# jameshensman/pyvb

Measured on AMD Instinct MI355X. Metric: VB update iterations/sec (T=10k, D=64, N=1024 LDS); ELBO rel-err vs NumPy, higher is better.
Workload: dtype f64; 1 GPU; LDS T=10000 D=64 K=64, 1024 replicates per GPU (BASELINE configs[2]); replicates_total=1024, parallelism=replicates sharded over 1 GPU(s), collective=none (1 GPU), degraded=False

## Files before the change

### pyvb_amd/csrc/k_cols.hip

```cpp
#include "params.h"

#define MFMA(a, b, c) __builtin_amdgcn_mfma_f64_16x16x4f64((a), (b), (c), 0, 0, 0)
#define MS 72
#define GS 68

__device__ __forceinline__ void load_row16(const double* row, int col0, int D, bool vec, double fill, double* out) {
    if (vec) {
#pragma unroll
        for (int g = 0; g < 4; ++g) {
            if (col0 + 4 * g < D) {
                const d4 v = *reinterpret_cast<const d4*>(row + col0 + 4 * g);
                out[4 * g] = v[0]; out[4 * g + 1] = v[1]; out[4 * g + 2] = v[2]; out[4 * g + 3] = v[3];
            } else {
                out[4 * g] = out[4 * g + 1] = out[4 * g + 2] = out[4 * g + 3] = fill;
            }
        }
    } else {
#pragma unroll
        for (int u = 0; u < 16; ++u) {
            const int c = col0 + u;
            const double v = row[c < D ? c : D - 1];
            out[u] = c < D ? v : fill;
        }
    }
}

__global__ void __launch_bounds__(64) k_cols(ParamArgs a) {
    const int WHICH = a.which0 + blockIdx.y;
    __shared__ double Mb[64 * MS];
    __shared__ double Gb[16 * GS];
    __shared__ double Sb[16 * GS];
    const int n = blockIdx.x, lane = threadIdx.x, D = a.D, K = a.K, c = lane & 15, q = lane >> 4;
    if (!a.active[n]) return;
    const int rows = WHICH == 0 ? D : K;
    double* M = (WHICH == 0 ? a.A_mean : a.C_mean) + (size_t)n * rows * D;
    double* V = (WHICH == 0 ? a.A_var : a.C_var) + (size_t)n * D * rows;
    double* qld = (WHICH == 0 ? a.qld_A : a.qld_C) + (size_t)n * D;
    double* lnd = (WHICH == 0 ? a.lnd_A : a.lnd_C) + (size_t)n * D;
    const double* pm = WHICH == 0 ? a.pri.A_pm : a.pri.C_pm;
    const double* pp = WHICH == 0 ? a.pri.A_pp : a.pri.C_pp;
    const double* obs = WHICH == 0 ? a.pri.A_obs : a.pri.C_obs;
    const double* mo = a.mom + (size_t)n * mom_total(D, K);
    const double* G = mo + (WHICH == 0 ? MOM_GA(D, K) : MOM_GC(D, K));
    const double* H = mo + (WHICH == 0 ? MOM_HA(D, K) : MOM_HC(D, K));
    const bool live = lane < rows;
    const int lr = live ? lane : 0;
    const int lc = lane < D ? lane : D - 1;
    const bool vec = (D & 3) == 0;
    const int nb = (D + 15) >> 4;
    const double* Mrow = M + (size_t)lr * D;
    const double* Hrow = H + (size_t)lr * D;

    for (int b = 0; b < 4; ++b) {
        double m[16] = {};
        if (b < nb) load_row16(Mrow, 16 * b, D, vec, 0.0, m);
#pragma unroll
        for (int u = 0; u < 16; ++u) Mb[(16 * b + u) * MS + lane] = (b < nb && live) ? m[u] : 0.0;
    }
    const double lam = live ? (WHICH == 0 ? a.Q_a[(size_t)n * D + lane] / a.Q_b[(size_t)n * D + lane]
                                          : a.R_a[(size_t)n * K + lane] / a.R_b[(size_t)n * K + lane]) : 0.0;

    auto stage_G = [&](int b) {
        double g[16];
#pragma unroll
        for (int u = 0; u < 16; ++u) {
            const int i = 16 * b + u;
            g[u] = G[(size_t)(i < D ? i : D - 1) * D + lc];
        }
#pragma unroll
        for (int u = 0; u < 16; ++u) Gb[u * GS + lane] = (16 * b + u < D && lane < D) ? g[u] : 0.0;
    };
    auto product = [&]() {
        d4 acc[4];
#pragma unroll
        for (int rt = 0; rt < 4; ++rt) acc[rt] = d4{0.0, 0.0, 0.0, 0.0};
#pragma unroll 4
        for (int s = 0; s < 16; ++s) {
            const double bop = Gb[c * GS + 4 * s + q];
#pragma unroll
            for (int rt = 0; rt < 4; ++rt) acc[rt] = MFMA(Mb[(4 * s + q) * MS + 16 * rt + c], bop, acc[rt]);
        }
#pragma unroll
        for (int rt = 0; rt < 4; ++rt)
#pragma unroll
            for (int r = 0; r < 4; ++r) Sb[c * GS + 16 * rt + 4 * r + q] = acc[rt][r];
    };

    if (a.c0 < a.c1) {
        for (int b = a.c0 >> 4; b <= (a.c1 - 1) >> 4; ++b) {
            __syncthreads();
            stage_G(b);
            double p0[16], m0[16], hk[16], ob[16];
#pragma unroll
            for (int u = 0; u < 16; ++u) {
                const int i = 16 * b + u;
                p0[u] = pp[(size_t)(i < D ? i : D - 1) * rows + lr];
            }
            load_row16(pm + (size_t)lr * D, 16 * b, D, vec, 0.0, m0);
            load_row16(Hrow, 16 * b, D, vec, 0.0, hk);
            load_row16(obs + (size_t)lr * D, 16 * b, D, vec, 0.0, ob);
            __syncthreads();
            product();
            __syncthreads();
            double gd[16], var[16], base[16];
#pragma unroll
            for (int u = 0; u < 16; ++u) {
                gd[u] = Gb[u * GS + 16 * b + u];
                const double prec = p0[u] + lam * gd[u];
                var[u] = 1.0 / prec;
                base[u] = p0[u] * m0[u] + lam * hk[u];
                p0[u] = prec;
            }
            double dl[16];
            int mynk = 0;
#pragma unroll
            for (int u = 0; u < 16; ++u) {
                const int i = 16 * b + u;
                dl[u] = 0.0;
                if (i >= a.c0 && i < a.c1) {
                    const double xo = Mb[i * MS + lane];
                    double acc = Sb[u * GS + lane] - xo * gd[u];
#pragma unroll
                    for (int v = 0; v < u; ++v) acc += dl[v] * Gb[u * GS + 16 * b + v];
                    double val = (base[u] - lam * acc) * var[u], vr = var[u];
                    const bool known = live && (ob[u] == ob[u]);
                    if (known) { val = ob[u]; vr = 0.0; }
                    const int nknown = __popcll(__ballot(known));
                    mynk = (lane == u) ? nknown : mynk;
                    if (live) {
                        dl[u] = val - xo;
                        Mb[i * MS + lane] = val;
                        V[(size_t)i * rows + lane] = vr;
                    }
                    Sb[u * GS + lane] = live ? p0[u] : 1.0;
                } else {
                    Sb[u * GS + lane] = 1.0;
                    mynk = (lane == u) ? rows : mynk;
                }
            }
            __syncthreads();
            {
                double mant = 1.0; int ex = 0;
#pragma unroll
                for (int r = 0; r < 16; ++r) {
                    int e;
                    mant *= frexp(Sb[c * GS + 16 * q + r], &e);
                    ex += e;
                }
#pragma unroll
                for (int o = 16; o <= 32; o <<= 1) {
                    mant *= __shfl_xor(mant, o, 64);
                    ex += __shfl_xor(ex, o, 64);
                }
                const int i = 16 * b + c;
                if (q == 0 && i >= a.c0 && i < a.c1 && mynk < rows) {
                    const double lp = log(mant) + (double)ex * 0.6931471805599453;
                    qld[i] = 0.5 / (0.5 * lp);
                    lnd[i] = -lp;
                }
            }
        }
        __syncthreads();
        if (live) {
            for (int b = a.c0 >> 4; b <= (a.c1 - 1) >> 4; ++b) {
#pragma unroll
                for (int g = 0; g < 4; ++g) {
                    const int cc = 16 * b + 4 * g;
                    if (vec) {
                        if (cc < D) {
                            d4 v;
#pragma unroll
                            for (int r = 0; r < 4; ++r) v[r] = Mb[(cc + r) * MS + lane];
                            *reinterpret_cast<d4*>(M + (size_t)lane * D + cc) = v;
                        }
                    } else {
#pragma unroll
                        for (int r = 0; r < 4; ++r)
                            if (cc + r < D) M[(size_t)lane * D + cc + r] = Mb[(cc + r) * MS + lane];
                    }
                }
            }
        }
    }

    if (a.fuse & 1) {
        double e0 = 0.0, e1 = 0.0, hm0 = 0.0, hm1 = 0.0;
        for (int b = 0; b < nb; ++b) {
            __syncthreads();
            stage_G(b);
            double hk[16], vv[16];
            load_row16(Hrow, 16 * b, D, vec, 0.0, hk);
#pragma unroll
            for (int u = 0; u < 16; ++u) {
                const int i = 16 * b + u;
                vv[u] = V[(size_t)(i < D ? i : D - 1) * rows + lr];
            }
            __syncthreads();
            product();
            __syncthreads();
#pragma unroll
            for (int u = 0; u < 16; u += 2) {
                const int i = 16 * b + u;
                const double x0 = Mb[i * MS + lane], x1 = Mb[(i + 1) * MS + lane];
                e0 += x0 * Sb[u * GS + lane] + (i < D ? vv[u] * Gb[u * GS + i] : 0.0);
                e1 += x1 * Sb[(u + 1) * GS + lane] + (i + 1 < D ? vv[u + 1] * Gb[(u + 1) * GS + i + 1] : 0.0);
                hm0 += x0 * hk[u];
                hm1 += x1 * hk[u + 1];
            }
        }
        const double own = WHICH == 0 ? mo[MOM_DP(D, K) + lr] : a.Syy[(size_t)n * K + lr];
        double r = 0.5 * own + 0.5 * (e0 + e1) - (hm0 + hm1);
        if (live) (WHICH == 0 ? a.resQ : a.resR)[(size_t)n * rows + lane] = r;
        if (a.fuse & 2) {
            const double* b0 = WHICH == 0 ? a.pri.Q_b0 : a.pri.R_b0;
            double* qb = (WHICH == 0 ? a.Q_b : a.R_b) + (size_t)n * rows;
            r = live ? r : 0.0;
            if (a.noise == PYVB_NOISE_GAMMA) {
                r = wave_sum(r);
                if (live) qb[lane] = b0[0] + r;
            } else if (live) {
                qb[lane] = b0[lane] + r;
            }
        }
    }
}

int launch_cols(pyvb_lds* h, int which, int c0, int c1, int fuse) {
    if (h->big) return launch_cols_big(h, which, c0, c1, fuse);
    ParamArgs a = make_args(h);
    a.c0 = c0; a.c1 = c1; a.which0 = which == 1 ? 1 : 0; a.fuse = fuse;
    TimedLaunch tl(h, PYVB_K_PARAMS);
    hipLaunchKernelGGL(k_cols, dim3(h->N, which == 2 ? 2 : 1), dim3(64), 0, h->stream, a);
    HIPCHK(hipGetLastError());
    return PYVB_OK;
}

int launch_resid(pyvb_lds* h, int which) { return launch_cols(h, which, 0, 0, 1); }
```

Before: 87.57 VB iterations/s per 1024 replicates (whole job).

## Hold mean matrix in MFMA-operand registers, staging only a 16-column tile in LDS

The full 64x64 mean matrix now lives in per-lane registers laid out as MFMA A operands, instead of a 64-row LDS buffer. Only the current 16-column block is copied into a small LDS tile for the sequential coordinate update, then copied back into registers and written to global memory per block. This cuts LDS use (more blocks per CU) and replaces LDS operand reads in the matrix product with register reads. The cost is 64 extra VGPRs per lane, register select logic in to_tile/from_tile, and a fully unrolled product loop, which may raise register pressure or cause spills.

Result: no change. 88.40 VB iterations/s per 1024 replicates (whole job), median of 6 (+1.0%).

```diff
diff --git a/pyvb_amd/csrc/k_cols.hip b/pyvb_amd/csrc/k_cols.hip
--- a/pyvb_amd/csrc/k_cols.hip
+++ b/pyvb_amd/csrc/k_cols.hip
@@ -27,7 +27,7 @@
 
 __global__ void __launch_bounds__(64) k_cols(ParamArgs a) {
     const int WHICH = a.which0 + blockIdx.y;
-    __shared__ double Mb[64 * MS];
+    __shared__ double Tb[16 * MS];
     __shared__ double Gb[16 * GS];
     __shared__ double Sb[16 * GS];
     const int n = blockIdx.x, lane = threadIdx.x, D = a.D, K = a.K, c = lane & 15, q = lane >> 4;
@@ -48,15 +48,36 @@
     const int lc = lane < D ? lane : D - 1;
     const bool vec = (D & 3) == 0;
     const int nb = (D + 15) >> 4;
-    const double* Mrow = M + (size_t)lr * D;
     const double* Hrow = H + (size_t)lr * D;
 
-    for (int b = 0; b < 4; ++b) {
-        double m[16] = {};
-        if (b < nb) load_row16(Mrow, 16 * b, D, vec, 0.0, m);
-#pragma unroll
-        for (int u = 0; u < 16; ++u) Mb[(16 * b + u) * MS + lane] = (b < nb && live) ? m[u] : 0.0;
-    }
+    double Mr[4][16];
+#pragma unroll
+    for (int rt = 0; rt < 4; ++rt)
+#pragma unroll
+        for (int s = 0; s < 16; ++s) {
+            const int r = 16 * rt + c, j = 4 * s + q;
+            const double v = M[(size_t)(r < rows ? r : rows - 1) * D + (j < D ? j : D - 1)];
+            Mr[rt][s] = __longlong_as_double(__double_as_longlong(v) & ((r < rows && j < D) ? -1ll : 0ll));
+        }
+    auto to_tile = [&](int b) {
+#pragma unroll
+        for (int sl = 0; sl < 4; ++sl)
+#pragma unroll
+            for (int rt = 0; rt < 4; ++rt) {
+                const double lo = b == 0 ? Mr[rt][sl] : Mr[rt][4 + sl], hi = b == 2 ? Mr[rt][8 + sl] : Mr[rt][12 + sl];
+                Tb[(4 * sl + q) * MS + 16 * rt + c] = b < 2 ? lo : hi;
+            }
+    };
+    auto from_tile = [&](int b) {
+#pragma unroll
+        for (int sl = 0; sl < 4; ++sl)
+#pragma unroll
+            for (int rt = 0; rt < 4; ++rt) {
+                const double t = Tb[(4 * sl + q) * MS + 16 * rt + c];
+#pragma unroll
+                for (int bb = 0; bb < 4; ++bb) Mr[rt][4 * bb + sl] = bb == b ? t : Mr[rt][4 * bb + sl];
+            }
+    };
     const double lam = live ? (WHICH == 0 ? a.Q_a[(size_t)n * D + lane] / a.Q_b[(size_t)n * D + lane]
                                           : a.R_a[(size_t)n * K + lane] / a.R_b[(size_t)n * K + lane]) : 0.0;
 
@@ -74,11 +95,11 @@
         d4 acc[4];
 #pragma unroll
         for (int rt = 0; rt < 4; ++rt) acc[rt] = d4{0.0, 0.0, 0.0, 0.0};
-#pragma unroll 4
+#pragma unroll
         for (int s = 0; s < 16; ++s) {
             const double bop = Gb[c * GS + 4 * s + q];
 #pragma unroll
-            for (int rt = 0; rt < 4; ++rt) acc[rt] = MFMA(Mb[(4 * s + q) * MS + 16 * rt + c], bop, acc[rt]);
+            for (int rt = 0; rt < 4; ++rt) acc[rt] = MFMA(Mr[rt][s], bop, acc[rt]);
         }
 #pragma unroll
         for (int rt = 0; rt < 4; ++rt)
@@ -90,6 +111,7 @@
         for (int b = a.c0 >> 4; b <= (a.c1 - 1) >> 4; ++b) {
             __syncthreads();
             stage_G(b);
+            to_tile(b);
             double p0[16], m0[16], hk[16], ob[16];
 #pragma unroll
             for (int u = 0; u < 16; ++u) {
@@ -118,7 +140,7 @@
                 const int i = 16 * b + u;
                 dl[u] = 0.0;
                 if (i >= a.c0 && i < a.c1) {
-                    const double xo = Mb[i * MS + lane];
+                    const double xo = Tb[u * MS + lane];
                     double acc = Sb[u * GS + lane] - xo * gd[u];
 #pragma unroll
                     for (int v = 0; v < u; ++v) acc += dl[v] * Gb[u * GS + 16 * b + v];
@@ -129,7 +151,7 @@
                     mynk = (lane == u) ? nknown : mynk;
                     if (live) {
                         dl[u] = val - xo;
-                        Mb[i * MS + lane] = val;
+                        Tb[u * MS + lane] = val;
                         V[(size_t)i * rows + lane] = vr;
                     }
                     Sb[u * GS + lane] = live ? p0[u] : 1.0;
@@ -159,10 +181,8 @@
                     lnd[i] = -lp;
                 }
             }
-        }
-        __syncthreads();
-        if (live) {
-            for (int b = a.c0 >> 4; b <= (a.c1 - 1) >> 4; ++b) {
+            from_tile(b);
+            if (live) {
 #pragma unroll
                 for (int g = 0; g < 4; ++g) {
                     const int cc = 16 * b + 4 * g;
@@ -170,13 +190,13 @@
                         if (cc < D) {
                             d4 v;
 #pragma unroll
-                            for (int r = 0; r < 4; ++r) v[r] = Mb[(cc + r) * MS + lane];
+                            for (int r = 0; r < 4; ++r) v[r] = Tb[(4 * g + r) * MS + lane];
                             *reinterpret_cast<d4*>(M + (size_t)lane * D + cc) = v;
                         }
                     } else {
 #pragma unroll
                         for (int r = 0; r < 4; ++r)
-                            if (cc + r < D) M[(size_t)lane * D + cc + r] = Mb[(cc + r) * MS + lane];
+                            if (cc + r < D) M[(size_t)lane * D + cc + r] = Tb[(4 * g + r) * MS + lane];
                     }
                 }
             }
@@ -188,6 +208,7 @@
         for (int b = 0; b < nb; ++b) {
             __syncthreads();
             stage_G(b);
+            to_tile(b);
             double hk[16], vv[16];
             load_row16(Hrow, 16 * b, D, vec, 0.0, hk);
 #pragma unroll
@@ -201,7 +222,7 @@
 #pragma unroll
             for (int u = 0; u < 16; u += 2) {
                 const int i = 16 * b + u;
-                const double x0 = Mb[i * MS + lane], x1 = Mb[(i + 1) * MS + lane];
+                const double x0 = Tb[u * MS + lane], x1 = Tb[(u + 1) * MS + lane];
                 e0 += x0 * Sb[u * GS + lane] + (i < D ? vv[u] * Gb[u * GS + i] : 0.0);
                 e1 += x1 * Sb[(u + 1) * GS + lane] + (i + 1 < D ? vv[u + 1] * Gb[(u + 1) * GS + i + 1] : 0.0);
                 hm0 += x0 * hk[u];
```
